# MaxMax2016/MixGAN-TTS

Hardware: AMD Instinct MI355X
Metric: denoiser steps/sec (80-mel, L=1000 frames, B=16 per GPU) (higher is better)
Workload: dtype f32

## Files before the change

include/mixgan_hip.h:

```cpp
#ifndef MIXGAN_HIP_H
#define MIXGAN_HIP_H

#include <stddef.h>
#include <stdint.h>

#ifdef __cplusplus
extern "C" {
#endif

#define MG_OK 0
#define MG_ERR_ARG (-1)
#define MG_ERR_SHAPE (-2)
#define MG_ERR_WORKSPACE (-3)

#define MG_VERSION 100

int mg_version(void);
const char *mg_error_string(int code);

#define MG_ACT_NONE 0
#define MG_ACT_RELU 1
#define MG_ACT_LRELU02 2
#define MG_ACT_TANH 3
#define MG_ACT_LRELU 4
// ... 19 lines not shown
int mg_conv1d_wgrad(const float *dy, const float *x, const float *x_vec, float *dw, float *scratch,
                    int B, int Co, int Ci, int Ldy, int Lx, int K, int stride, int pad, float alpha,
                    int accumulate, void *stream);

int mg_conv1d_wgrad_strided(const float *dy, long dy_bs, const float *x, long x_bs, const float *x_vec,
                            float *dw, float *scratch, int B, int Co, int Ci, int Ldy, int Lx, int K,
                            int stride, int pad, float alpha, int accumulate, void *stream);

size_t mg_conv1d_wgrad_grouped_scratch_floats(int Co, int Ci, int K, int G);
int mg_conv1d_wgrad_grouped(const float *dy, long dy_bs, long dy_gs, const float *x, long x_bs, long x_gs, float *dw,
                            long dw_gs, float *scratch, int G, int B, int Co, int Ci, int Ldy, int Lx, int K, int stride,
                            int pad, float alpha, int accumulate, void *stream);
int mg_conv1d_wgrad_grouped_bias(const float *dy, long dy_bs, long dy_gs, const float *x, long x_bs, long x_gs, float *dw,
                                 long dw_gs, float *db, long db_gs, float *scratch, int G, int B, int Co, int Ci, int Ldy,
                                 int Lx, int K, int stride, int pad, float alpha, int accumulate, void *stream);

int mg_rowsum(const float *in, long in_bs, int B, int R, int L, float *out_r, float *out_br,
              float alpha, int accumulate, void *stream);

int mg_conv1d_fwd_ex(const float *in, const float *in_vec, const float *packed, const float *bias,
                     const float *add, float *out, int B, int Ci, int Lin, int Co, int Lout, int K,
                     int stride, int pad, int dil, float in_slope, int act, float act_slope, float alpha,
                     int accumulate, void *stream);
int mg_conv1d_fwd_split(const float *in, const float *in_vec, const float *packed, const float *bias,
                        const float *add, float *out, int B, int Ci, int Lin, int Co, int Lout, int K, int stride,
                        int pad, int dil, float in_slope, int act, float act_slope, float alpha, int accumulate,
                        float *scratch, size_t scratch_floats, void *stream);

#define MG_CONV_EPI_PLAIN 0
#define MG_CONV_EPI_REFLECT 1
// ... 377 lines not shown
```

mixgan-tts_amd/_lib.py:

```python
import ctypes
import os
import subprocess

import torch

_HERE = os.path.dirname(os.path.abspath(__file__))
_LIB = None

class MixganHipError(RuntimeError):
    pass


MG_OK, MG_ERR_ARG, MG_ERR_SHAPE, MG_ERR_WORKSPACE = 0, -1, -2, -3
MG_ACT_NONE, MG_ACT_RELU, MG_ACT_LRELU02, MG_ACT_TANH, MG_ACT_LRELU = range(5)
MG_PACK_PLAIN, MG_PACK_GATE, MG_PACK_DGRAD, MG_PACK_TPOSE, MG_PACK_PLAIN16, MG_PACK_GATE16 = range(6)
MG_DEN_BACKWARD, MG_DEN_SPLIT, MG_DEN_P16, MG_DEN_JOBS_RESIDENT = 1, 2, 4, 8
MG_FWD_SAVE, MG_FWD_SPLIT, MG_FWD_P16 = 1, 2, 4
MG_PLAN_PER_LAYER, MG_PLAN_SINGLE = 0, 1
MG_PLAN_PERSIST, MG_PLAN_PERSIST16, MG_PLAN_TEAM16 = 0, 1, 2
MG_STATUS_TICKET, MG_STATUS_ERROR, MG_STATUS_LAUNCHES, MG_STATUS_DONE, MG_STATUS_WORDS = range(5)
MG_CONV_EPI_PLAIN, MG_CONV_EPI_REFLECT, MG_CONV_EPI_PHASES_SLICE, MG_CONV_EPI_NEEDS_WM2 = range(4)
MG_DEN_HEAD_PTRS, MG_DEN_LAYER_PTRS = 8, 9
(MG_DEN_IN_W, MG_DEN_IN_B, MG_DEN_MLP0_W, MG_DEN_MLP2_W, MG_DEN_SKIP_W, MG_DEN_SKIP_B, MG_DEN_OUT_W,
 MG_DEN_OUT_B) = range(MG_DEN_HEAD_PTRS)
# ... 18 lines not shown
                ("mel_bins", ctypes.c_int32), ("multi_speaker", ctypes.c_int32)]


class SamplingLoop(ctypes.Structure):
    _fields_ = [("cproj", ctypes.c_void_p), ("cproj_out", ctypes.c_void_p), ("step_vectors", ctypes.c_void_p),
                ("step_index", ctypes.c_int32), ("step_count", ctypes.c_int32)]


class FwdPlan(ctypes.Structure):
    _fields_ = [(n, ctypes.c_int32) for n in ("path", "family", "nt", "waves", "solo", "team", "cproj_mode", "grid",
                                              "block")]


class ConvPlan(ctypes.Structure):
    _fields_ = [(n, ctypes.c_int32) for n in ("kw", "stride", "ck", "dilmax", "mw", "wm", "nnb", "ksplit", "grid")]


def library_path():
    return os.environ.get("MG_HIP_LIB") or os.path.join(_HERE, "libmixgan_hip.so")


def build(force=False):
    if force or not os.path.exists(library_path()):
        subprocess.check_call(["make", "-C", os.path.join(_HERE, "csrc"), "-j4"] + (["-B"] if force else []))
    return library_path()


def lib():
    global _LIB
    if _LIB is None:
# ... 35 lines not shown
        "mg_conv_transpose_pack": (i, [vp, vp, i, i, i, vp]),
        "mg_conv_transpose1d_fwd": (i, [vp, vp, vp, vp, i, i, i, i, i, f, f, vp]),
        "mg_diffuse_fwd": (i, [vp] * 9 + [i, i, i, i, vp]),
        "mg_posterior_sample_fwd": (i, [vp] * 10 + [i, i, i, i, i, vp]),
        "mg_transpose_bml": (i, [vp] * 5 + [i, i, i, i, i, vp]),
        "mg_posterior_sample_bwd": (i, [vp] * 7 + [i, i, i, i, i, vp]),
        "mg_spec_affine": (i, [vp, vp, vp, vp, i, sz, i, vp]),
        "mg_conv_pack_at": (i, [vp, vp, i, i, i, i, i, i, vp]),
        "mg_conv1d_wgrad_scratch_floats": (sz, [i, i, i]),
        "mg_conv1d_wgrad": (i, [vp, vp, vp, vp, vp, i, i, i, i, i, i, i, i, f, i, vp]),
        "mg_conv1d_wgrad_strided": (i, [vp, lg, vp, lg, vp, vp, vp, i, i, i, i, i, i, i, i, f, i, vp]),
        "mg_rowsum": (i, [vp, lg, i, i, i, vp, vp, f, i, vp]),
        "mg_conv1d_wgrad_grouped_scratch_floats": (sz, [i, i, i, i]),
        "mg_conv1d_wgrad_grouped": (i, [vp, lg, lg, vp, lg, lg, vp, lg, vp, i, i, i, i, i, i, i, i, i, f, i, vp]),
        "mg_conv1d_wgrad_grouped_bias": (i, [vp, lg, lg, vp, lg, lg, vp, lg, vp, lg, vp, i, i, i, i, i, i, i, i, i, f, i, vp]),
        "mg_denoiser_packed_floats": (sz, [dp, i]),
        "mg_denoiser_pack": (i, [dp, vp, vp, vp, i, vp]),
        "mg_denoiser_bwd_workspace_floats": (sz, [dp, i, i]),
        "mg_denoiser_bwd": (i, [dp, vp, vp, vp, vp, vp, vp, vp, sz, vp, vp, vp, vp, i, i, vp]),
        "mg_denoiser_bwd_staged": (i, [dp, vp, vp, vp, vp, vp, vp, vp, sz, vp, vp, vp, vp, i, i, vp, vp]),
        "mg_denoiser_workspace_floats": (sz, [dp, i, i, i]),
        "mg_denoiser_fwd": (i, [dp, vp, vp, vp, vp, vp, vp, vp, sz, i, i, i, vp]),
        "mg_denoiser_fwd_pair": (i, [dp, vp, vp, vp, vp, vp, vp, vp, vp, vp, vp, vp, vp, sz, vp, sz, i, i, vp]),
        "mg_denoiser_fwd_plan": (i, [dp, i, i, i, i, i, ctypes.POINTER(FwdPlan)]),
        "mg_transpose_bml_strided": (i, [vp] * 5 + [i, i, i, i, i, lg, vp]),
        "mg_act_bwd": (i, [vp, vp, vp, i, sz, vp]),
        "mg_upsample_zero": (i, [vp, vp, i, i, i, i, vp]),
        "mg_step_mlp_fwd": (i, [vp] * 8 + [i, i, i, i, vp]),
        "mg_step_mlp_bwd": (i, [vp] * 8 + [i, i, i, i, vp]),
        "mg_linear_small_fwd": (i, [vp, vp, vp, i, i, i, vp]),
# ... 125 lines not shown
```

mixgan-tts_amd/autograd.py:

```python
import torch

from . import ops, _lib


def _require_cuda(*ts):
    for t in ts:
        if t is not None and not t.is_cuda:
            raise _lib.MixganHipError("tensor on %s: the HIP path has no CPU fallback" % t.device)


class _TransposeFn(torch.autograd.Function):

    @staticmethod
    def forward(ctx, x, to_blm):
        ctx.to_blm = to_blm
        return ops.transpose_bml(x.contiguous(), to_blm)

    @staticmethod
    def backward(ctx, g):
        return ops.transpose_bml(g.contiguous(), not ctx.to_blm), None


def transpose_to_bml(x):
    _require_cuda(x)
# ... 75 lines not shown
        ctx.through = through_posterior
        ctx.mark_non_differentiable(xpp) if not through_posterior else None
        return x0c, xpp

    @staticmethod
    def backward(ctx, g_x0c, g_xpp):
        x0, t, keep, c1 = ctx.saved_tensors
        g = ops.posterior_sample_bwd(x0, t, keep, c1, g_x0c.contiguous(),
                                     g_xpp.contiguous() if ctx.through else None, ctx.clip)
        return (g,) + (None,) * 9


class _Conv1dFn(torch.autograd.Function):

    @staticmethod
    def forward(ctx, x, weight, bias, in_vec, stride, padding, act):
        _require_cuda(x)
        x = x.contiguous()
        Co, Ci, K = weight.shape
        y = ops.conv1d_packed(x, ops.pack_cached(weight), None if bias is None else bias.detach(), Co, K, stride,
                              padding, act, in_vec=None if in_vec is None else in_vec.detach().contiguous(), split=True)
        ctx.save_for_backward(x, weight, y if act else None, in_vec)
        ctx.cfg = (stride, padding, act, bias is not None)
        return y

    @staticmethod
    def backward(ctx, gy):
        x, weight, y, in_vec = ctx.saved_tensors
        stride, padding, act, has_bias = ctx.cfg
        Co, Ci, K = weight.shape
        gy = gy.contiguous()
        dpre = ops.act_bwd(gy, y, act) if act else gy
        need = ctx.needs_input_grad
        vec = None if in_vec is None else in_vec.detach().contiguous()
        dw = ops.conv1d_wgrad(dpre, x, K, stride, padding, x_vec=vec) if need[1] else None
        db = ops.rowsum(dpre) if (has_bias and need[2]) else None
        dx = dvec = None
        if need[0] or (in_vec is not None and need[3]):
            Lin = x.shape[2]
            src = dpre
            if stride > 1:
                src = ops.upsample_zero(dpre, stride, (dpre.shape[2] - 1) * stride + 1)
            dx = ops.conv1d_packed(src, ops.pack_cached(weight, ops.PACK_DGRAD), None, Ci, K, 1, K - 1 - padding,
                                   Lout=Lin, split=True)
            if in_vec is not None and need[3]:
                dvec = ops.rowsum(dx, per_batch=True)
        return dx if need[0] else None, dw, db, dvec, None, None, None


def conv1d(x, weight, bias=None, stride=1, padding=0, act=None, in_vec=None):
    return _Conv1dFn.apply(x, weight, bias, in_vec, stride, padding, act)


class _StepMlpFn(torch.autograd.Function):
    @staticmethod
    def forward(ctx, t, freq, W0, W2):
        out, emb, pre, h = ops.step_mlp_fwd(t.contiguous(), freq, W0.detach().contiguous(), W2.detach().contiguous())
        ctx.save_for_backward(emb, pre, h, W2)
        return out

    @staticmethod
    def backward(ctx, g):
        emb, pre, h, W2 = ctx.saved_tensors
        dW0, dW2 = ops.step_mlp_bwd(g.contiguous(), emb, pre, h, W2.detach().contiguous())
        return None, None, dW0, dW2

# ... 189 lines not shown
```

mixgan-tts_amd/csrc/conv_api.hip:

```cpp
#include "conv_mfma.h"
#include "wgrad_mfma.h"

__global__ void pack_conv_kernel(const float *__restrict__ w, float *__restrict__ wp, PackDesc d)
{
    const size_t total = (size_t)d.MB * (d.CiP * d.K / 8) * 256;
    for (size_t idx = (size_t)blockIdx.x * blockDim.x + threadIdx.x; idx < total; idx += (size_t)gridDim.x * blockDim.x) {
        size_t dst;
        const float v = mg_pack_element(w, d, idx, &dst);
        wp[dst] = v;
    }
}

extern "C" size_t mg_conv_packed_floats(int Co, int Ci, int K, int mode)
{
    int Mrows, Kin, MB;
    if (pack_dims(Co, Ci, K, mode, &Mrows, &Kin, &MB) != MG_OK) return 0;
    const int CiP = mg_round_up(Kin, mg_conv_ck(K));
    return (size_t)MB * (CiP * K / 8) * 256;
}

extern "C" int mg_conv_pack_at(const float *w, float *packed, int Co, int Ci, int K, int mode, int q0, int Qtot,
                               void *stream)
{
    if (!w || !packed) return MG_ERR_ARG;
// ... 167 lines not shown
                               int Co, int Ci, int Ldy, int Lx, int K, int stride, int pad, float alpha,
                               int accumulate, void *stream)
{
    return mg_conv1d_wgrad_strided(dy, 0, x, 0, x_vec, dw, scratch, B, Co, Ci, Ldy, Lx, K, stride, pad, alpha, accumulate,
                                   stream);
}

__global__ __launch_bounds__(256) void rowsum_kernel(const float *__restrict__ in, long in_bs, int B, int R, int L,
                                                     float *__restrict__ out_r, float *__restrict__ out_br,
                                                     float alpha, int accumulate, int vec4)
{
    __shared__ float red[4];
    const int r = blockIdx.x;
    const int lane = threadIdx.x & 63, wave = threadIdx.x >> 6;
    if (!out_br) {
        float v = 0.f;
        if (vec4) {
            const int L4 = L >> 2;
            for (int b = 0; b < B; ++b) {
                const f32x4 *p = reinterpret_cast<const f32x4 *>(in + (size_t)b * in_bs + (size_t)r * L);
                for (int l = threadIdx.x; l < L4; l += 256) {
                    const f32x4 q = p[l];
                    v += (q[0] + q[1]) + (q[2] + q[3]);
                }
            }
        } else {
            for (int b = 0; b < B; ++b) {
                const float *p = in + (size_t)b * in_bs + (size_t)r * L;
                for (int l = threadIdx.x; l < L; l += 256) v += p[l];
            }
        }
#pragma unroll
        for (int o = 32; o > 0; o >>= 1) v += __shfl_xor(v, o, 64);
        if (lane == 0) red[wave] = v;
        __syncthreads();
        if (threadIdx.x == 0) {
            const float tot = alpha * (red[0] + red[1] + red[2] + red[3]);
            out_r[r] = accumulate ? out_r[r] + tot : tot;
        }
        return;
    }
    float tot = 0.f;
    for (int b = 0; b < B; ++b) {
        const float *p = in + (size_t)b * in_bs + (size_t)r * L;
        float v = 0.f;
        for (int l = threadIdx.x; l < L; l += 256) v += p[l];
#pragma unroll
        for (int o = 32; o > 0; o >>= 1) v += __shfl_xor(v, o, 64);
        __syncthreads();
        if (lane == 0) red[wave] = v;
        __syncthreads();
        const float s = red[0] + red[1] + red[2] + red[3];
        if (threadIdx.x == 0) out_br[(size_t)b * R + r] = alpha * s;
        tot += s;
    }
    if (out_r && threadIdx.x == 0) out_r[r] = accumulate ? out_r[r] + alpha * tot : alpha * tot;
}

extern "C" int mg_rowsum(const float *in, long in_bs, int B, int R, int L, float *out_r, float *out_br, float alpha,
                         int accumulate, void *stream)
{
    if (!in || (!out_r && !out_br)) return MG_ERR_ARG;
    if (B <= 0 || R <= 0 || L <= 0) return MG_ERR_SHAPE;
    const long bs = in_bs ? in_bs : (long)R * L;
    const int vec4 = (L % 4 == 0) && (bs % 4 == 0) && (((uintptr_t)in & 15) == 0);
    hipLaunchKernelGGL(rowsum_kernel, dim3(R), dim3(256), 0, (hipStream_t)stream, in, bs, B, R, L, out_r, out_br, alpha,
                       accumulate, vec4);
    MG_LAUNCH_CHECK();
    return MG_OK;
}
```

mixgan-tts_amd/csrc/wgrad_mfma.h:

```cpp
#pragma once
#include "common.h"
#include "wgrad_stream.h"
#include <cstdlib>

#define WG_FT 64
#define WG_RSA 65
#define WG_RSB 73

struct WgradArgs {
    const float *dy;
    const float *x;
    const float *xvec;
    float *scratch;
    long dy_bs, x_bs;
    int B, Co, Ci, Ldy, Lx, K, stride, pad;
    int chunks_per_b, nchunks, nsplit, ci_tiles;
    int G;
    long dy_gs, x_gs;
};

template <bool VEC>
__global__ __launch_bounds__(256, 2) void wgrad_mfma_kernel(WgradArgs a)
{
    __shared__ float lds[128 * WG_RSA + 128 * WG_RSB];
    float *ldsA = lds, *ldsB = lds + 128 * WG_RSA;

    const int tid = threadIdx.x;
    const int lane = tid & 63;
    const int wave = tid >> 6;
    const int wm = wave >> 1, wn = wave & 1;
    const int hh = lane >> 5, c32 = lane & 31;
    const int split = blockIdx.x;
    const int co0 = (blockIdx.y / a.ci_tiles) * 128;
    const int ci0 = (blockIdx.y % a.ci_tiles) * 128;
    const int grp = blockIdx.z / a.K;
    const int tap = blockIdx.z - grp * a.K;

    f32x16 acc[2][2];
#pragma unroll
    for (int i = 0; i < 2; ++i)
#pragma unroll
        for (int j = 0; j < 2; ++j)
#pragma unroll
            for (int r = 0; r < 16; ++r) acc[i][j][r] = 0.f;

    f32x4 va[VEC ? 8 : 1], vb[VEC ? 9 : 1];
    float sa[VEC ? 1 : 8], sb[VEC ? 1 : 8];
    const int shift = tap - a.pad;
    const int shift4 = shift & ~3, rsh = VEC ? (shift & 3) : 0;
    const int c4A = tid & 15;
    int gA[VEC ? 8 : 1], gB[VEC ? 9 : 1], lB[VEC ? 9 : 1], c4B[VEC ? 9 : 1];
// ... 120 lines not shown
    float *dst = a.scratch + (((size_t)split * a.G + grp) * a.K + tap) * a.Co * a.Ci;
#pragma unroll
    for (int i = 0; i < 2; ++i)
#pragma unroll
        for (int r = 0; r < 16; ++r) {
            const int co = co0 + wm * 64 + i * 32 + 8 * (r >> 2) + 4 * hh + (r & 3);
            if (co >= a.Co) continue;
#pragma unroll
            for (int j = 0; j < 2; ++j) {
                const int ci = ci0 + wn * 64 + j * 32 + c32;
                if (ci < a.Ci) dst[(size_t)co * a.Ci + ci] = acc[i][j][r];
            }
        }
}

__global__ __launch_bounds__(256) void wgrad_finalize_kernel(const float *__restrict__ scratch, float *__restrict__ dw,
                                                             int Co, int Ci, int K, int G, long dw_gs, int nsplit,
                                                             float alpha, int accumulate)
{
    __shared__ float part[8][32];
    const size_t per = (size_t)Co * Ci * K, n = per * G;
    const int lane = threadIdx.x & 31, grp = threadIdx.x >> 5;
    for (size_t base = (size_t)blockIdx.x * 32; base < n; base += (size_t)gridDim.x * 32) {
        const size_t i = base + lane;
        float v0 = 0.f, v1 = 0.f;
        if (i < n) {
            int s = grp;
            for (; s + 8 < nsplit; s += 16) {
                v0 += scratch[(size_t)s * n + i];
                v1 += scratch[(size_t)(s + 8) * n + i];
            }
            if (s < nsplit) v0 += scratch[(size_t)s * n + i];
        }
        part[grp][lane] = v0 + v1;
        __syncthreads();
        if (grp == 0 && i < n) {
            float v = part[0][lane];
#pragma unroll
            for (int q = 1; q < 8; ++q) v += part[q][lane];
            v *= alpha;
            const size_t g = i / per, r = i - g * per;
            const size_t cc = r % ((size_t)Co * Ci);
            const int k = (int)(r / ((size_t)Co * Ci));
            float *o = dw + g * dw_gs + cc * K + k;
            *o = accumulate ? *o + v : v;
        }
        __syncthreads();
    }
}

static inline int wgrad_nsplit(int Co, int Ci, int K, int G = 1)
{
    const int tiles = mg_cdiv(Co, 128) * mg_cdiv(Ci, 128) * K * G;
    const int target = tiles <= 8 ? 256 : 512;
    const int n = target / tiles;
    return n < 1 ? 1 : n;
}
static inline size_t wgrad_scratch_floats(int Co, int Ci, int K, int G = 1)
{
    const size_t split = (size_t)wgrad_nsplit(Co, Ci, K, G) * G * Co * Ci * K;
    const size_t stream = wgrad_stream_scratch_floats(Co, Ci, K, G);
    return split > stream ? split : stream;
}

struct WgradShape {
    int B, Co, Ci, Ldy, Lx, K, stride, pad;
    long dy_bs, x_bs;
    int G = 1;
    long dy_gs = 0, x_gs = 0, dw_gs = 0;
    float *db = nullptr;
    long db_gs = 0;
    bool *db_done = nullptr;
};

static int wgrad_launch(const WgradShape &s, const float *dy, const float *x, const float *xvec, float *dw,
                        float *scratch, float alpha, int accumulate, hipStream_t st)
{
    if (s.B <= 0 || s.Co <= 0 || s.Ci <= 0 || s.Ldy <= 0 || s.Lx <= 0 || s.K <= 0 || s.G <= 0) return MG_ERR_SHAPE;
    WgradArgs a;
    a.G = s.G;
    a.dy_gs = s.dy_gs;
    a.x_gs = s.x_gs;
    a.dy = dy;
    a.x = x;
    a.xvec = xvec;
    a.scratch = scratch;
    a.dy_bs = s.dy_bs ? s.dy_bs : (long)s.Co * s.Ldy;
    a.x_bs = s.x_bs ? s.x_bs : (long)s.Ci * s.Lx;
    a.B = s.B;
    a.Co = s.Co;
    a.Ci = s.Ci;
    a.Ldy = s.Ldy;
    a.Lx = s.Lx;
    a.K = s.K;
    a.stride = s.stride;
    a.pad = s.pad;
    a.chunks_per_b = mg_cdiv(s.Ldy, WG_FT);
    a.nchunks = a.chunks_per_b * s.B;
    a.ci_tiles = mg_cdiv(s.Ci, 128);
    int nsplit = wgrad_nsplit(s.Co, s.Ci, s.K, s.G);
    if (nsplit > a.nchunks) nsplit = a.nchunks;
    a.nsplit = nsplit;
    const size_t n = (size_t)s.Co * s.Ci * s.K * s.G;
    dim3 grid(nsplit, mg_cdiv(s.Co, 128) * a.ci_tiles, s.K * s.G);
    {
        const char *env = std::getenv("MG_WGRAD_STREAM");
        const bool stream_on = !(env && env[0] == '0');
        const long dybs = a.dy_bs, xbs = a.x_bs;
        const WsShape w = wgrad_stream_shape(s.Co, s.Ci, s.K);
        const long long units = w.cfg ? (long long)wgrad_stream_tiles(w, s.Co, s.Ci, s.G) * s.B * mg_cdiv(s.Ldy, w.FT) : 0;
        const bool ok = stream_on && w.cfg && s.stride == 1 && !xvec && s.pad == (s.K - 1) / 2 && s.Ldy == s.Lx &&
                        s.Ldy % 4 == 0 && s.Ldy >= 4 && dybs % 4 == 0 && xbs % 4 == 0 && s.dy_gs % 4 == 0 &&
                        s.x_gs % 4 == 0 && ((((uintptr_t)dy | (uintptr_t)x) & 15) == 0) && units * 2 < (1ll << 31) &&
                        units >= 8 * WS_NW;
        if (ok) {
            if (s.db_done) *s.db_done = s.db != nullptr;
            return wgrad_stream_launch(w, dy, x, dw, scratch, s.G, s.B, s.Co, s.Ci, s.Ldy, dybs, xbs, s.dy_gs, s.x_gs,
                                       s.dw_gs ? s.dw_gs : (long)s.Co * s.Ci * s.K, alpha, accumulate, st, s.db, s.db_gs);
        }
    }
    const bool vec = s.stride == 1 && !xvec && (s.Ldy % 4 == 0) && (s.Lx % 4 == 0) && (a.dy_bs % 4 == 0) &&
                     (a.x_bs % 4 == 0) && (a.dy_gs % 4 == 0) && (a.x_gs % 4 == 0) && ((((uintptr_t)dy | (uintptr_t)x) & 15) == 0) && s.Ldy >= 4 && s.Lx >= 4;
    if (vec) hipLaunchKernelGGL(wgrad_mfma_kernel<true>, grid, dim3(256), 0, st, a);
    else hipLaunchKernelGGL(wgrad_mfma_kernel<false>, grid, dim3(256), 0, st, a);
    MG_LAUNCH_CHECK();
    const int blocks = (int)((n + 31) / 32 < 8192 ? (n + 31) / 32 : 8192);
    hipLaunchKernelGGL(wgrad_finalize_kernel, dim3(blocks), dim3(256), 0, st, scratch, dw, s.Co, s.Ci, s.K, s.G,
                       s.dw_gs ? s.dw_gs : (long)s.Co * s.Ci * s.K, nsplit, alpha, accumulate);
    MG_LAUNCH_CHECK();
    return MG_OK;
}
```

mixgan-tts_amd/discriminator.py:

```python
import os

import torch
from torch import nn

from . import autograd as A
from .blocks import ConvNorm, LinearNorm, DiffusionEmbedding, Mish


class JCUDiscriminator(nn.Module):

    def __init__(self, preprocess_config, model_config, train_config):
        super().__init__()
        n_mel_channels = preprocess_config["preprocessing"]["mel"]["n_mel_channels"]
        residual_channels = model_config["denoiser"]["residual_channels"]
        dc = model_config["discriminator"]
        n_layer, n_uncond_layer, n_cond_layer = dc["n_layer"], dc["n_uncond_layer"], dc["n_cond_layer"]
        n_channels, kernel_sizes, strides = dc["n_channels"], dc["kernel_sizes"], dc["strides"]
        self.multi_speaker = model_config["multi_speaker"]

        self.input_projection = LinearNorm(2 * n_mel_channels, 2 * n_mel_channels)
        self.diffusion_embedding = DiffusionEmbedding(residual_channels)
        self.mlp = nn.Sequential(
            LinearNorm(residual_channels, residual_channels * 4),
            Mish(),
# ... 4 lines not shown

        def conv(i):
            return ConvNorm(n_channels[i - 1] if i != 0 else 2 * n_mel_channels, n_channels[i],
                            kernel_size=kernel_sizes[i], stride=strides[i], dilation=1)

        self.conv_block = nn.ModuleList([conv(i) for i in range(n_layer)])
        self.uncond_conv_block = nn.ModuleList([conv(i) for i in range(n_layer, n_layer + n_uncond_layer)])
        self.cond_conv_block = nn.ModuleList([conv(i) for i in range(n_layer, n_layer + n_cond_layer)])
        self.apply(self.weights_init)
        self._freq = None

    def weights_init(self, m):
        if m.__class__.__name__.find("ConvNorm") != -1:
            m.conv.weight.data.normal_(0.0, 0.02)

    @staticmethod
    def _lrelu_conv(layer, x, in_vec=None):
        return A.conv1d(x, layer.conv.weight, layer.conv.bias, layer.stride, layer.padding, "lrelu", in_vec)

    def forward(self, x_ts, x_t_prevs, s, t):
        dev = x_ts.device
        if self._freq is None or self._freq.device != dev:
            self._freq = self.diffusion_embedding.frequencies(dev).contiguous()
        x = A.cat_transpose(x_t_prevs, x_ts)
        x = A.conv1d(x, self.input_projection.linear.weight[:, :, None], None)
        step = A.step_mlp(t, self._freq, self.mlp[0].linear.weight, self.mlp[2].linear.weight)
        if self.multi_speaker:
            step = step + A.linear_small(s, self.spk_mlp[0].linear.weight)
        cond_feats, uncond_feats = [], []
        for layer in self.conv_block:
            x = self._lrelu_conv(layer, x)
            cond_feats.append(x)
            uncond_feats.append(x)
        x_cond, x_uncond = x, x
        overlap = (self.branch_overlap and os.environ.get("MG_JCU_OVERLAP", "1") != "0" and x.is_cuda
                   and not torch.cuda.is_current_stream_capturing())
        if overlap:
            main = torch.cuda.current_stream(dev)
            if self._side is None or self._side.device != dev:
                self._side = torch.cuda.Stream(device=dev)
# ... 22 lines not shown
```

mixgan-tts_amd/ops.py:

```python
import ctypes
import os

import torch

from . import _lib
from ._lib import fptr, iptr, check, stream_ptr

ACT = {None: _lib.MG_ACT_NONE, "none": _lib.MG_ACT_NONE, "relu": _lib.MG_ACT_RELU, "lrelu": _lib.MG_ACT_LRELU02,
       "tanh": _lib.MG_ACT_TANH, "lrelu_s": _lib.MG_ACT_LRELU}
PACK_PLAIN, PACK_GATE, PACK_DGRAD = _lib.MG_PACK_PLAIN, _lib.MG_PACK_GATE, _lib.MG_PACK_DGRAD


def pack_conv_weight(w, mode=PACK_PLAIN, out=None):
    L = _lib.lib()
    if w.dim() == 2:
        w = w[:, :, None]
    w = w.detach().contiguous()
    Co, Ci, K = w.shape
    n = L.mg_conv_packed_floats(Co, Ci, K, mode)
    if n == 0:
        raise _lib.MixganHipError("unsupported conv weight shape %s" % (tuple(w.shape),))
    if out is None or out.numel() != n or out.device != w.device:
        out = torch.empty(n, device=w.device, dtype=torch.float32)
    check(L.mg_conv_pack(fptr(w), fptr(out), Co, Ci, K, mode, stream_ptr()))
# ... 134 lines not shown
    out = torch.empty_like(x)
    check(L.mg_spec_affine(fptr(x), fptr(out), fptr(spec_min.reshape(-1)), fptr(spec_max.reshape(-1)), mode,
                           x.numel(), M, stream_ptr()))
    return out


def conv1d_wgrad(dy, x, K, stride=1, padding=0, x_vec=None, alpha=1.0):
    L = _lib.lib()
    B, Co, Ldy = dy.shape
    _, Ci, Lx = x.shape
    dw = torch.empty(Co, Ci, K, device=x.device, dtype=torch.float32)
    scratch = torch.empty(L.mg_conv1d_wgrad_scratch_floats(Co, Ci, K), device=x.device, dtype=torch.float32)
    check(L.mg_conv1d_wgrad(fptr(dy), fptr(x), fptr(x_vec, True), fptr(dw), fptr(scratch), B, Co, Ci, Ldy, Lx, K,
                            stride, padding, float(alpha), 0, stream_ptr()))
    return dw


def rowsum(x, per_batch=False, alpha=1.0):
    L = _lib.lib()
    B, R, Lf = x.shape
    out = torch.empty((B, R) if per_batch else (R,), device=x.device, dtype=torch.float32)
    check(L.mg_rowsum(fptr(x), 0, B, R, Lf, fptr(None if per_batch else out, True), fptr(out if per_batch else None, True),
                      float(alpha), 0, stream_ptr()))
    return out


def act_bwd(dy, y, act):
    L = _lib.lib()
    out = torch.empty_like(dy)
    check(L.mg_act_bwd(fptr(dy), fptr(y), fptr(out), ACT[act], dy.numel(), stream_ptr()))
# ... 254 lines not shown
```

mixgan-tts_amd/train_step.py:

```python
import os

import torch

from . import losses
from .distributed import GradBucket, ShardCounts, exchange_batch_shape, is_distributed
from .optimizer import FlatAdam


class HotPathTrainer:
    def __init__(self, diffusion, discriminator, train_config, model_config, extra_g_params=(), g_param_order=None,
                 resume=None, first_step=1, exact_shards=False):
        self.G, self.D = diffusion, discriminator
        self.exact_shards = bool(exact_shards)
        oc = train_config["optimizer"]
        self.grad_clip = oc["grad_clip_thresh"]
        self.lambda_fm = train_config["loss"]["lambda_fm" if diffusion.model != "shallow" else "lambda_fm_shallow"]
        self.n_layers = model_config["discriminator"]["n_layer"] + model_config["discriminator"]["n_cond_layer"]
        self.grad_acc = int(oc.get("grad_acc_step", 1))
        if self.grad_acc < 1:
            raise ValueError("grad_acc_step must be >= 1")
        self.step_no = int(first_step)
        g_params = list(diffusion.parameters()) + list(extra_g_params)
        self.bucketG = GradBucket(g_params, order=diffusion.denoise_fn.grad_order())
        self.bucketD = GradBucket(list(discriminator.parameters()))
        order_g = list(g_param_order) if g_param_order is not None else g_params
        if self.bucketG.flat.is_cuda:
            diffusion.denoise_fn.bind_grad_buffer(self.bucketG.flat, self.bucketG.offsets)
            self.optG = FlatAdam(self.bucketG, lr=oc["init_lr_G"], betas=oc["betas"], param_order=order_g)
            self.optD = FlatAdam(self.bucketD, lr=oc["init_lr_D"], betas=oc["betas"],
                                 param_order=list(discriminator.parameters()))
        else:
            self.optG = torch.optim.Adam(order_g, lr=oc["init_lr_G"], betas=oc["betas"])
            self.optD = torch.optim.Adam(discriminator.parameters(), lr=oc["init_lr_D"], betas=oc["betas"])
        if resume is not None:
            for mine, theirs in ((self.optG, resume[0]), (self.optD, resume[1])):
                if isinstance(mine, FlatAdam):
                    mine.adopt(theirs)
                else:
                    mine.load_state_dict(theirs.state_dict())
        self.sdlG = torch.optim.lr_scheduler.ExponentialLR(self.optG, gamma=oc["gamma"])
        self.sdlD = torch.optim.lr_scheduler.ExponentialLR(self.optD, gamma=oc["gamma"])
        if resume is not None:
            self.sdlG.load_state_dict(resume[2].state_dict())
            self.sdlD.load_state_dict(resume[3].state_dict())
        self.d_loss_fn, self.g_loss_fn = losses.get_adversarial_losses_fn(train_config["loss"]["adv_loss_mode"])
# ... 408 lines not shown
```

Before: 373.1.

## Batch discriminator conv weight-gradients into grouped multi-job MFMA kernel launches

Discriminator convolutions defer their weight and bias gradient work to a group that is flushed at the end of backward. The flush launches a single job-table MFMA wgrad kernel plus one finalize kernel that also does the bias rowsums, instead of separate wgrad and rowsum launches per layer. Gradients are written straight into the flat gradient bucket views, which saves extra allocations and copies. This removes per-layer launch overhead and raises GPU occupancy for the small wgrad problems, at the cost of extra Python bookkeeping, cross-stream waits and a deferred callback.

```diff
diff --git a/include/mixgan_hip.h b/include/mixgan_hip.h
--- a/include/mixgan_hip.h
+++ b/include/mixgan_hip.h
@@ -57,6 +57,16 @@
 int mg_conv1d_wgrad_grouped_bias(const float *dy, long dy_bs, long dy_gs, const float *x, long x_bs, long x_gs, float *dw,
                                  long dw_gs, float *db, long db_gs, float *scratch, int G, int B, int Co, int Ci, int Ldy,
                                  int Lx, int K, int stride, int pad, float alpha, int accumulate, void *stream);
+
+typedef struct mg_wgrad_job {
+    const float *dy, *x, *x_vec;
+    float *dw, *db;
+    int B, Co, Ci, Ldy, Lx, K, stride, pad;
+    float alpha;
+    int accumulate, db_accumulate;
+} mg_wgrad_job;
+size_t mg_conv1d_wgrad_jobs_scratch_floats(const mg_wgrad_job *jobs, int n);
+int mg_conv1d_wgrad_jobs(const mg_wgrad_job *jobs, int n, float *scratch, void *stream);
 
 int mg_rowsum(const float *in, long in_bs, int B, int R, int L, float *out_r, float *out_br,
               float alpha, int accumulate, void *stream);
diff --git a/mixgan-tts_amd/_lib.py b/mixgan-tts_amd/_lib.py
--- a/mixgan-tts_amd/_lib.py
+++ b/mixgan-tts_amd/_lib.py
@@ -56,6 +56,12 @@
 
 class ConvPlan(ctypes.Structure):
     _fields_ = [(n, ctypes.c_int32) for n in ("kw", "stride", "ck", "dilmax", "mw", "wm", "nnb", "ksplit", "grid")]
+
+
+class WgradJob(ctypes.Structure):
+    _fields_ = ([(n, ctypes.c_void_p) for n in ("dy", "x", "x_vec", "dw", "db")] +
+                [(n, ctypes.c_int32) for n in ("B", "Co", "Ci", "Ldy", "Lx", "K", "stride", "pad")] +
+                [("alpha", ctypes.c_float), ("accumulate", ctypes.c_int32), ("db_accumulate", ctypes.c_int32)])
 
 
 def library_path():
@@ -121,6 +127,8 @@
         "mg_conv1d_wgrad_grouped_scratch_floats": (sz, [i, i, i, i]),
         "mg_conv1d_wgrad_grouped": (i, [vp, lg, lg, vp, lg, lg, vp, lg, vp, i, i, i, i, i, i, i, i, i, f, i, vp]),
         "mg_conv1d_wgrad_grouped_bias": (i, [vp, lg, lg, vp, lg, lg, vp, lg, vp, lg, vp, i, i, i, i, i, i, i, i, i, f, i, vp]),
+        "mg_conv1d_wgrad_jobs_scratch_floats": (sz, [ctypes.POINTER(WgradJob), i]),
+        "mg_conv1d_wgrad_jobs": (i, [ctypes.POINTER(WgradJob), i, vp, vp]),
         "mg_denoiser_packed_floats": (sz, [dp, i]),
         "mg_denoiser_pack": (i, [dp, vp, vp, vp, i, vp]),
         "mg_denoiser_bwd_workspace_floats": (sz, [dp, i, i]),
diff --git a/mixgan-tts_amd/autograd.py b/mixgan-tts_amd/autograd.py
--- a/mixgan-tts_amd/autograd.py
+++ b/mixgan-tts_amd/autograd.py
@@ -113,7 +113,7 @@
 class _Conv1dFn(torch.autograd.Function):
 
     @staticmethod
-    def forward(ctx, x, weight, bias, in_vec, stride, padding, act):
+    def forward(ctx, x, weight, bias, in_vec, stride, padding, act, member=None):
         _require_cuda(x)
         x = x.contiguous()
         Co, Ci, K = weight.shape
@@ -121,6 +121,7 @@
                               padding, act, in_vec=None if in_vec is None else in_vec.detach().contiguous(), split=True)
         ctx.save_for_backward(x, weight, y if act else None, in_vec)
         ctx.cfg = (stride, padding, act, bias is not None)
+        ctx.member = member
         return y
 
     @staticmethod
@@ -132,8 +133,13 @@
         dpre = ops.act_bwd(gy, y, act) if act else gy
         need = ctx.needs_input_grad
         vec = None if in_vec is None else in_vec.detach().contiguous()
-        dw = ops.conv1d_wgrad(dpre, x, K, stride, padding, x_vec=vec) if need[1] else None
-        db = ops.rowsum(dpre) if (has_bias and need[2]) else None
+        if ctx.member is not None and need[1]:
+            group, wparam, bparam = ctx.member
+            group.add(dpre, x, vec, wparam, bparam if (has_bias and need[2]) else None, stride, padding)
+            dw = db = None
+        else:
+            dw = ops.conv1d_wgrad(dpre, x, K, stride, padding, x_vec=vec) if need[1] else None
+            db = ops.rowsum(dpre) if (has_bias and need[2]) else None
         dx = dvec = None
         if need[0] or (in_vec is not None and need[3]):
             Lin = x.shape[2]
@@ -144,11 +150,86 @@
                                    Lout=Lin, split=True)
             if in_vec is not None and need[3]:
                 dvec = ops.rowsum(dx, per_batch=True)
-        return dx if need[0] else None, dw, db, dvec, None, None, None
-
-
-def conv1d(x, weight, bias=None, stride=1, padding=0, act=None, in_vec=None):
-    return _Conv1dFn.apply(x, weight, bias, in_vec, stride, padding, act)
+        return dx if need[0] else None, dw, db, dvec, None, None, None, None
+
+
+def conv1d(x, weight, bias=None, stride=1, padding=0, act=None, in_vec=None, member=None):
+    return _Conv1dFn.apply(x, weight, bias, in_vec, stride, padding, act, member)
+
+
+class WgradGroup:
+
+    def __init__(self):
+        self.jobs = []
+
+    @staticmethod
+    def set_home(param, view):
+        param.__dict__["_mg_grad_home"] = view
+
+    def reset(self):
+        self.jobs = []
+
+    def add(self, dy, x, x_vec, wparam, bparam, stride, padding):
+        if not self.jobs:
+            torch.autograd.Variable._execution_engine.queue_callback(self.flush)
+        self.jobs.append((dy, x, x_vec, wparam, bparam, stride, padding, torch.cuda.current_stream(dy.device)))
+
+    @staticmethod
+    def _target(p):
+        g = p.grad
+        if g is None:
+            home = p.__dict__.get("_mg_grad_home")
+            if home is None or home.shape != p.shape or home.device != p.device:
+                home = torch.empty(p.shape, device=p.device, dtype=torch.float32)
+            p.grad = home
+            return home, False, None
+        if g.dtype == torch.float32 and g.is_contiguous() and g.device == p.device:
+            return g, True, None
+        tmp = torch.empty(p.shape, device=p.device, dtype=torch.float32)
+        return tmp, False, tmp
+
+    def flush(self):
+        jobs, self.jobs = self.jobs, []
+        if not jobs:
+            return
+        dev = jobs[0][0].device
+        with torch.no_grad(), torch.cuda.device(dev):
+            cur = torch.cuda.current_stream(dev)
+            waited = set()
+            for (dy, x, x_vec, _, _, _, _, stream) in jobs:
+                if stream != cur:
+                    if stream.cuda_stream not in waited and not torch.cuda.is_current_stream_capturing():
+                        cur.wait_stream(stream)
+                    waited.add(stream.cuda_stream)
+                    for t in (dy, x, x_vec):
+                        if t is not None:
+                            t.record_stream(cur)
+            waves, last = [], {}
+            for job in jobs:
+                w = 1 + max([last.get(id(p), -1) for p in job[3:5] if p is not None])
+                for p in job[3:5]:
+                    if p is not None:
+                        last[id(p)] = w
+                if w == len(waves):
+                    waves.append([])
+                waves[w].append(job)
+            for wave in waves:
+                table, later = [], []
+                for (dy, x, x_vec, wp, bp, stride, padding, _) in wave:
+                    dw, acc, add_w = self._target(wp)
+                    job = {"dy": dy, "x": x, "x_vec": x_vec, "dw": dw, "accumulate": acc, "stride": stride,
+                           "padding": padding}
+                    if add_w is not None:
+                        later.append((wp, add_w))
+                    if bp is not None:
+                        db, dacc, add_b = self._target(bp)
+                        job["db"], job["db_accumulate"] = db, dacc
+                        if add_b is not None:
+                            later.append((bp, add_b))
+                    table.append(job)
+                ops.conv1d_wgrad_jobs(table)
+                for p, t in later:
+                    p.grad = p.grad + t.to(p.grad.dtype).view_as(p.grad)
 
 
 class _StepMlpFn(torch.autograd.Function):
diff --git a/mixgan-tts_amd/csrc/conv_api.hip b/mixgan-tts_amd/csrc/conv_api.hip
--- a/mixgan-tts_amd/csrc/conv_api.hip
+++ b/mixgan-tts_amd/csrc/conv_api.hip
@@ -205,30 +205,8 @@
     const int r = blockIdx.x;
     const int lane = threadIdx.x & 63, wave = threadIdx.x >> 6;
     if (!out_br) {
-        float v = 0.f;
-        if (vec4) {
-            const int L4 = L >> 2;
-            for (int b = 0; b < B; ++b) {
-                const f32x4 *p = reinterpret_cast<const f32x4 *>(in + (size_t)b * in_bs + (size_t)r * L);
-                for (int l = threadIdx.x; l < L4; l += 256) {
-                    const f32x4 q = p[l];
-                    v += (q[0] + q[1]) + (q[2] + q[3]);
-                }
-            }
-        } else {
-            for (int b = 0; b < B; ++b) {
-                const float *p = in + (size_t)b * in_bs + (size_t)r * L;
-                for (int l = threadIdx.x; l < L; l += 256) v += p[l];
-            }
-        }
-#pragma unroll
-        for (int o = 32; o > 0; o >>= 1) v += __shfl_xor(v, o, 64);
-        if (lane == 0) red[wave] = v;
-        __syncthreads();
-        if (threadIdx.x == 0) {
-            const float tot = alpha * (red[0] + red[1] + red[2] + red[3]);
-            out_r[r] = accumulate ? out_r[r] + tot : tot;
-        }
+        const float tot = alpha * rowsum_row_total(in, in_bs, B, L, r, vec4, red);
+        if (threadIdx.x == 0) out_r[r] = accumulate ? out_r[r] + tot : tot;
         return;
     }
     float tot = 0.f;
@@ -254,9 +232,50 @@
     if (!in || (!out_r && !out_br)) return MG_ERR_ARG;
     if (B <= 0 || R <= 0 || L <= 0) return MG_ERR_SHAPE;
     const long bs = in_bs ? in_bs : (long)R * L;
-    const int vec4 = (L % 4 == 0) && (bs % 4 == 0) && (((uintptr_t)in & 15) == 0);
+    const int vec4 = rowsum_vec4(in, bs, L);
     hipLaunchKernelGGL(rowsum_kernel, dim3(R), dim3(256), 0, (hipStream_t)stream, in, bs, B, R, L, out_r, out_br, alpha,
                        accumulate, vec4);
     MG_LAUNCH_CHECK();
     return MG_OK;
 }
+
+static WgradJob wgrad_job_of(const mg_wgrad_job &j)
+{
+    return WgradJob{j.dy, j.x, j.x_vec, j.dw, j.db, j.B, j.Co, j.Ci, j.Ldy, j.Lx, j.K, j.stride, j.pad, j.alpha,
+                    j.accumulate, j.db_accumulate};
+}
+
+extern "C" size_t mg_conv1d_wgrad_jobs_scratch_floats(const mg_wgrad_job *jobs, int n)
+{
+    if (!jobs || n <= 0) return 0;
+    size_t tot = WG_TABLE_FLOATS;
+    for (int i = 0; i < n; ++i) {
+        if (jobs[i].Co <= 0 || jobs[i].Ci <= 0 || jobs[i].K <= 0) return 0;
+        tot += wgrad_job_scratch_floats(wgrad_job_of(jobs[i]));
+    }
+    return tot;
+}
+
+extern "C" int mg_conv1d_wgrad_jobs(const mg_wgrad_job *jobs, int n, float *scratch, void *stream)
+{
+    if (!jobs || !scratch) return MG_ERR_ARG;
+    if (n <= 0) return MG_ERR_SHAPE;
+    float *sc = scratch + WG_TABLE_FLOATS;
+    for (int at = 0; at < n; at += WG_MAX_JOBS) {
+        const int m = n - at < WG_MAX_JOBS ? n - at : WG_MAX_JOBS;
+        WgradJob batch[WG_MAX_JOBS];
+        float *alone[WG_MAX_JOBS];
+        for (int i = 0; i < m; ++i) batch[i] = wgrad_job_of(jobs[at + i]);
+        MG_TRY(wgrad_jobs_batch(batch, m, scratch, sc, alone, (hipStream_t)stream));
+        for (int i = 0; i < m; ++i) {
+            const WgradJob &j = batch[i];
+            if (alone[i]) {
+                MG_TRY(mg_conv1d_wgrad(j.dy, j.x, j.xvec, j.dw, alone[i], j.B, j.Co, j.Ci, j.Ldy, j.Lx, j.K, j.stride, j.pad,
+                                       j.alpha, j.accumulate, stream));
+                if (j.db) MG_TRY(mg_rowsum(j.dy, 0, j.B, j.Co, j.Ldy, j.db, nullptr, j.alpha, j.db_accumulate, stream));
+            }
+            sc += wgrad_job_scratch_floats(j);
+        }
+    }
+    return MG_OK;
+}
diff --git a/mixgan-tts_amd/csrc/wgrad_mfma.h b/mixgan-tts_amd/csrc/wgrad_mfma.h
--- a/mixgan-tts_amd/csrc/wgrad_mfma.h
+++ b/mixgan-tts_amd/csrc/wgrad_mfma.h
@@ -19,10 +19,10 @@
     long dy_gs, x_gs;
 };
 
+#define WG_LDS_FLOATS (128 * WG_RSA + 128 * WG_RSB)
 template <bool VEC>
-__global__ __launch_bounds__(256, 2) void wgrad_mfma_kernel(WgradArgs a)
-{
-    __shared__ float lds[128 * WG_RSA + 128 * WG_RSB];
+__device__ __forceinline__ void wgrad_mfma_unit(const WgradArgs &a, float *lds, const int split, const int tile, const int z)
+{
     float *ldsA = lds, *ldsB = lds + 128 * WG_RSA;
 
     const int tid = threadIdx.x;
@@ -30,11 +30,10 @@
     const int wave = tid >> 6;
     const int wm = wave >> 1, wn = wave & 1;
     const int hh = lane >> 5, c32 = lane & 31;
-    const int split = blockIdx.x;
-    const int co0 = (blockIdx.y / a.ci_tiles) * 128;
-    const int ci0 = (blockIdx.y % a.ci_tiles) * 128;
-    const int grp = blockIdx.z / a.K;
-    const int tap = blockIdx.z - grp * a.K;
+    const int co0 = (tile / a.ci_tiles) * 128;
+    const int ci0 = (tile % a.ci_tiles) * 128;
+    const int grp = z / a.K;
+    const int tap = z - grp * a.K;
 
     f32x16 acc[2][2];
 #pragma unroll
@@ -185,14 +184,21 @@
         }
 }
 
-__global__ __launch_bounds__(256) void wgrad_finalize_kernel(const float *__restrict__ scratch, float *__restrict__ dw,
-                                                             int Co, int Ci, int K, int G, long dw_gs, int nsplit,
-                                                             float alpha, int accumulate)
-{
-    __shared__ float part[8][32];
+template <bool VEC>
+__global__ __launch_bounds__(256, 2) void wgrad_mfma_kernel(WgradArgs a)
+{
+    __shared__ float lds[WG_LDS_FLOATS];
+    wgrad_mfma_unit<VEC>(a, lds, blockIdx.x, blockIdx.y, blockIdx.z);
+}
+
+__device__ __forceinline__ void wgrad_finalize_blocks(const float *__restrict__ scratch, float *__restrict__ dw, int Co,
+                                                      int Ci, int K, int G, long dw_gs, int nsplit, float alpha,
+                                                      int accumulate, float (*part)[32], const unsigned blk,
+                                                      const unsigned nblk)
+{
     const size_t per = (size_t)Co * Ci * K, n = per * G;
     const int lane = threadIdx.x & 31, grp = threadIdx.x >> 5;
-    for (size_t base = (size_t)blockIdx.x * 32; base < n; base += (size_t)gridDim.x * 32) {
+    for (size_t base = (size_t)blk * 32; base < n; base += (size_t)nblk * 32) {
         const size_t i = base + lane;
         float v0 = 0.f, v1 = 0.f;
         if (i < n) {
@@ -217,6 +223,112 @@
             *o = accumulate ? *o + v : v;
         }
         __syncthreads();
+    }
+}
+
+__global__ __launch_bounds__(256) void wgrad_finalize_kernel(const float *__restrict__ scratch, float *__restrict__ dw,
+                                                             int Co, int Ci, int K, int G, long dw_gs, int nsplit,
+                                                             float alpha, int accumulate)
+{
+    __shared__ float part[8][32];
+    wgrad_finalize_blocks(scratch, dw, Co, Ci, K, G, dw_gs, nsplit, alpha, accumulate, part, blockIdx.x, gridDim.x);
+}
+
+__device__ __forceinline__ float rowsum_row_total(const float *__restrict__ in, long in_bs, int B, int L, int r, int vec4,
+                                                  float *red)
+{
+    const int lane = threadIdx.x & 63, wave = threadIdx.x >> 6;
+    float v = 0.f;
+    if (vec4) {
+        const int L4 = L >> 2;
+        for (int b = 0; b < B; ++b) {
+            const f32x4 *p = reinterpret_cast<const f32x4 *>(in + (size_t)b * in_bs + (size_t)r * L);
+            for (int l = threadIdx.x; l < L4; l += 256) {
+                const f32x4 q = p[l];
+                v += (q[0] + q[1]) + (q[2] + q[3]);
+            }
+        }
+    } else {
+        for (int b = 0; b < B; ++b) {
+            const float *p = in + (size_t)b * in_bs + (size_t)r * L;
+            for (int l = threadIdx.x; l < L; l += 256) v += p[l];
+        }
+    }
+#pragma unroll
+    for (int o = 32; o > 0; o >>= 1) v += __shfl_xor(v, o, 64);
+    if (lane == 0) red[wave] = v;
+    __syncthreads();
+    return red[0] + red[1] + red[2] + red[3];
+}
+static inline int rowsum_vec4(const float *in, long bs, int L) { return (L % 4 == 0) && (bs % 4 == 0) && (((uintptr_t)in & 15) == 0); }
+
+#define WG_MAX_JOBS 16
+struct WgradJobDev {
+    WgradArgs a;
+    float *dw, *db;
+    float alpha;
+    int accumulate, db_accumulate, db_vec4;
+    int ytiles;
+    int fin_blocks;
+    int vec;
+};
+struct WgradJobTable {
+    int nform[3];
+    int form_job[3][WG_MAX_JOBS];
+    int form_start[3][WG_MAX_JOBS + 1];
+    int nfin;
+    int fin_start[2 * WG_MAX_JOBS + 1];
+    WgradJobDev job[WG_MAX_JOBS];
+};
+static_assert(sizeof(WgradJobTable) <= 4000, "the table travels as a kernel argument");
+#define WG_TABLE_FLOATS ((sizeof(WgradJobTable) + 255) / 256 * 64)
+
+__device__ __forceinline__ int wgrad_job_search(const int *__restrict__ start, int n, int u)
+{
+    int lo = 0, hi = n;
+    while (hi - lo > 1) {
+        const int mid = (lo + hi) >> 1;
+        if (start[mid] <= u) lo = mid;
+        else hi = mid;
+    }
+    return lo;
+}
+
+__global__ __launch_bounds__(256) void wgrad_jobs_upload_kernel(WgradJobTable t, WgradJobTable *dst)
+{
+    const int *src = reinterpret_cast<const int *>(&t);
+    int *d = reinterpret_cast<int *>(dst);
+    for (unsigned i = threadIdx.x; i < sizeof(WgradJobTable) / 4; i += 256) d[i] = src[i];
+}
+
+template <int FORM>
+__global__ __launch_bounds__(256, 2) void wgrad_mfma_jobs_kernel(const WgradJobTable *__restrict__ t)
+{
+    __shared__ float lds[WG_LDS_FLOATS];
+    const int e = wgrad_job_search(t->form_start[FORM], t->nform[FORM], (int)blockIdx.x);
+    const WgradJobDev &j = t->job[t->form_job[FORM][e]];
+    const WgradArgs a = j.a;
+    int r = (int)blockIdx.x - t->form_start[FORM][e];
+    const int split = r % a.nsplit;
+    r /= a.nsplit;
+    const int tile = r % j.ytiles;
+    if (FORM == 1 || (FORM == 2 && j.vec)) wgrad_mfma_unit<true>(a, lds, split, tile, r / j.ytiles);
+    else wgrad_mfma_unit<false>(a, lds, split, tile, r / j.ytiles);
+}
+
+__global__ __launch_bounds__(256) void wgrad_finalize_jobs_kernel(const WgradJobTable *__restrict__ t)
+{
+    __shared__ float part[8][32];
+    __shared__ float red[4];
+    const int e = wgrad_job_search(t->fin_start, t->nfin, (int)blockIdx.x);
+    const WgradJobDev &j = t->job[e >> 1];
+    const unsigned local = blockIdx.x - t->fin_start[e];
+    if (!(e & 1)) {
+        wgrad_finalize_blocks(j.a.scratch, j.dw, j.a.Co, j.a.Ci, j.a.K, 1, (long)j.a.Co * j.a.Ci * j.a.K, j.a.nsplit, j.alpha,
+                              j.accumulate, part, local, (unsigned)j.fin_blocks);
+    } else {
+        const float tot = j.alpha * rowsum_row_total(j.a.dy, j.a.dy_bs, j.a.B, j.a.Ldy, (int)local, j.db_vec4, red);
+        if (threadIdx.x == 0) j.db[local] = j.db_accumulate ? j.db[local] + tot : tot;
     }
 }
 
@@ -244,11 +356,17 @@
     bool *db_done = nullptr;
 };
 
-static int wgrad_launch(const WgradShape &s, const float *dy, const float *x, const float *xvec, float *dw,
-                        float *scratch, float alpha, int accumulate, hipStream_t st)
+enum { WG_KIND_SCALAR = 0, WG_KIND_VEC = 1, WG_KIND_STREAM = 2 };
+struct WgradPlan {
+    WgradArgs a;
+    int kind;
+    WsShape w;
+    int ytiles, z;
+};
+static int wgrad_plan(const WgradShape &s, const float *dy, const float *x, const float *xvec, float *scratch, WgradPlan *p)
 {
     if (s.B <= 0 || s.Co <= 0 || s.Ci <= 0 || s.Ldy <= 0 || s.Lx <= 0 || s.K <= 0 || s.G <= 0) return MG_ERR_SHAPE;
-    WgradArgs a;
+    WgradArgs &a = p->a;
     a.G = s.G;
     a.dy_gs = s.dy_gs;
     a.x_gs = s.x_gs;
@@ -272,8 +390,8 @@
     int nsplit = wgrad_nsplit(s.Co, s.Ci, s.K, s.G);
     if (nsplit > a.nchunks) nsplit = a.nchunks;
     a.nsplit = nsplit;
-    const size_t n = (size_t)s.Co * s.Ci * s.K * s.G;
-    dim3 grid(nsplit, mg_cdiv(s.Co, 128) * a.ci_tiles, s.K * s.G);
+    p->ytiles = mg_cdiv(s.Co, 128) * a.ci_tiles;
+    p->z = s.K * s.G;
     {
         const char *env = std::getenv("MG_WGRAD_STREAM");
         const bool stream_on = !(env && env[0] == '0');
@@ -285,19 +403,130 @@
                         s.x_gs % 4 == 0 && ((((uintptr_t)dy | (uintptr_t)x) & 15) == 0) && units * 2 < (1ll << 31) &&
                         units >= 8 * WS_NW;
         if (ok) {
-            if (s.db_done) *s.db_done = s.db != nullptr;
-            return wgrad_stream_launch(w, dy, x, dw, scratch, s.G, s.B, s.Co, s.Ci, s.Ldy, dybs, xbs, s.dy_gs, s.x_gs,
-                                       s.dw_gs ? s.dw_gs : (long)s.Co * s.Ci * s.K, alpha, accumulate, st, s.db, s.db_gs);
+            p->kind = WG_KIND_STREAM;
+            p->w = w;
+            return MG_OK;
         }
     }
     const bool vec = s.stride == 1 && !xvec && (s.Ldy % 4 == 0) && (s.Lx % 4 == 0) && (a.dy_bs % 4 == 0) &&
                      (a.x_bs % 4 == 0) && (a.dy_gs % 4 == 0) && (a.x_gs % 4 == 0) && ((((uintptr_t)dy | (uintptr_t)x) & 15) == 0) && s.Ldy >= 4 && s.Lx >= 4;
-    if (vec) hipLaunchKernelGGL(wgrad_mfma_kernel<true>, grid, dim3(256), 0, st, a);
+    p->kind = vec ? WG_KIND_VEC : WG_KIND_SCALAR;
+    return MG_OK;
+}
+static inline int wgrad_finalize_grid(size_t n) { return (int)((n + 31) / 32 < 8192 ? (n + 31) / 32 : 8192); }
+
+static int wgrad_launch(const WgradShape &s, const float *dy, const float *x, const float *xvec, float *dw,
+                        float *scratch, float alpha, int accumulate, hipStream_t st)
+{
+    WgradPlan p;
+    MG_TRY(wgrad_plan(s, dy, x, xvec, scratch, &p));
+    const WgradArgs &a = p.a;
+    if (p.kind == WG_KIND_STREAM) {
+        if (s.db_done) *s.db_done = s.db != nullptr;
+        return wgrad_stream_launch(p.w, dy, x, dw, scratch, s.G, s.B, s.Co, s.Ci, s.Ldy, a.dy_bs, a.x_bs, s.dy_gs, s.x_gs,
+                                   s.dw_gs ? s.dw_gs : (long)s.Co * s.Ci * s.K, alpha, accumulate, st, s.db, s.db_gs);
+    }
+    const size_t n = (size_t)s.Co * s.Ci * s.K * s.G;
+    dim3 grid(a.nsplit, p.ytiles, p.z);
+    if (p.kind == WG_KIND_VEC) hipLaunchKernelGGL(wgrad_mfma_kernel<true>, grid, dim3(256), 0, st, a);
     else hipLaunchKernelGGL(wgrad_mfma_kernel<false>, grid, dim3(256), 0, st, a);
     MG_LAUNCH_CHECK();
-    const int blocks = (int)((n + 31) / 32 < 8192 ? (n + 31) / 32 : 8192);
-    hipLaunchKernelGGL(wgrad_finalize_kernel, dim3(blocks), dim3(256), 0, st, scratch, dw, s.Co, s.Ci, s.K, s.G,
-                       s.dw_gs ? s.dw_gs : (long)s.Co * s.Ci * s.K, nsplit, alpha, accumulate);
+    hipLaunchKernelGGL(wgrad_finalize_kernel, dim3(wgrad_finalize_grid(n)), dim3(256), 0, st, scratch, dw, s.Co, s.Ci, s.K,
+                       s.G, s.dw_gs ? s.dw_gs : (long)s.Co * s.Ci * s.K, a.nsplit, alpha, accumulate);
     MG_LAUNCH_CHECK();
     return MG_OK;
 }
+
+struct WgradJob {
+    const float *dy, *x, *xvec;
+    float *dw, *db;
+    int B, Co, Ci, Ldy, Lx, K, stride, pad;
+    float alpha;
+    int accumulate, db_accumulate;
+};
+static inline size_t wgrad_job_scratch_floats(const WgradJob &j)
+{
+    return (wgrad_scratch_floats(j.Co, j.Ci, j.K) + 63) / 64 * 64;
+}
+static int wgrad_jobs_batch(const WgradJob *jobs, int n, float *table, float *sc, float **alone, hipStream_t st)
+{
+    WgradJobTable t{};
+    WgradJobTable *dev = reinterpret_cast<WgradJobTable *>(table);
+    int work[WG_MAX_JOBS];
+    int nj = 0;
+    for (int i = 0; i < n; ++i) {
+        const WgradJob &j = jobs[i];
+        alone[i] = nullptr;
+        if (!j.dy || !j.x || !j.dw) return MG_ERR_ARG;
+        if (j.stride < 1 || j.pad < 0) return MG_ERR_SHAPE;
+        WgradShape s{j.B, j.Co, j.Ci, j.Ldy, j.Lx, j.K, j.stride, j.pad, 0, 0};
+        WgradPlan p;
+        MG_TRY(wgrad_plan(s, j.dy, j.x, j.xvec, sc, &p));
+        if (p.kind == WG_KIND_STREAM) {
+            alone[i] = sc;
+        } else {
+            WgradJobDev &d = t.job[nj];
+            d.a = p.a;
+            d.dw = j.dw;
+            d.db = j.db;
+            d.alpha = j.alpha;
+            d.accumulate = j.accumulate;
+            d.db_accumulate = j.db_accumulate;
+            d.db_vec4 = rowsum_vec4(j.dy, p.a.dy_bs, j.Ldy);
+            d.ytiles = p.ytiles;
+            d.fin_blocks = wgrad_finalize_grid((size_t)j.Co * j.Ci * j.K);
+            d.vec = p.kind == WG_KIND_VEC;
+            work[nj] = mg_cdiv(p.a.nchunks, p.a.nsplit);
+            for (int f = d.vec; f <= 2; f += 2 - d.vec) {
+                int at = t.nform[f]++;
+                while (at > 0 && work[t.form_job[f][at - 1]] < work[nj]) {
+                    t.form_job[f][at] = t.form_job[f][at - 1];
+                    --at;
+                }
+                t.form_job[f][at] = nj;
+            }
+            ++nj;
+        }
+        sc += wgrad_job_scratch_floats(j);
+    }
+    if (nj == 0) return MG_OK;
+    long long tot = 0;
+    for (int f = 0; f < 3; ++f) {
+        long long u = 0;
+        for (int e = 0; e < t.nform[f]; ++e) {
+            const WgradJobDev &d = t.job[t.form_job[f][e]];
+            t.form_start[f][e] = (int)u;
+            u += (long long)d.a.nsplit * d.ytiles * d.a.K;
+        }
+        if (u >= (1ll << 31)) return MG_ERR_SHAPE;
+        t.form_start[f][t.nform[f]] = (int)u;
+    }
+    t.nfin = 2 * nj;
+    for (int e = 0; e < nj; ++e) {
+        t.fin_start[2 * e] = (int)tot;
+        tot += t.job[e].fin_blocks;
+        t.fin_start[2 * e + 1] = (int)tot;
+        tot += t.job[e].db ? t.job[e].a.Co : 0;
+    }
+    if (tot >= (1ll << 31)) return MG_ERR_SHAPE;
+    t.fin_start[2 * nj] = (int)tot;
+    hipLaunchKernelGGL(wgrad_jobs_upload_kernel, dim3(1), dim3(256), 0, st, t, dev);
+    MG_LAUNCH_CHECK();
+    const char *env = std::getenv("MG_WGRAD_JOBS_GRIDS");
+    if (!(env && env[0] == '2') && t.nform[0] && t.nform[1]) {
+        hipLaunchKernelGGL(wgrad_mfma_jobs_kernel<2>, dim3(t.form_start[2][nj]), dim3(256), 0, st, dev);
+        MG_LAUNCH_CHECK();
+    } else {
+        if (t.nform[0]) {
+            hipLaunchKernelGGL(wgrad_mfma_jobs_kernel<0>, dim3(t.form_start[0][t.nform[0]]), dim3(256), 0, st, dev);
+            MG_LAUNCH_CHECK();
+        }
+        if (t.nform[1]) {
+            hipLaunchKernelGGL(wgrad_mfma_jobs_kernel<1>, dim3(t.form_start[1][t.nform[1]]), dim3(256), 0, st, dev);
+            MG_LAUNCH_CHECK();
+        }
+    }
+    hipLaunchKernelGGL(wgrad_finalize_jobs_kernel, dim3((unsigned)tot), dim3(256), 0, st, dev);
+    MG_LAUNCH_CHECK();
+    return MG_OK;
+}
diff --git a/mixgan-tts_amd/discriminator.py b/mixgan-tts_amd/discriminator.py
--- a/mixgan-tts_amd/discriminator.py
+++ b/mixgan-tts_amd/discriminator.py
@@ -42,16 +42,31 @@
         if m.__class__.__name__.find("ConvNorm") != -1:
             m.conv.weight.data.normal_(0.0, 0.02)
 
-    @staticmethod
-    def _lrelu_conv(layer, x, in_vec=None):
-        return A.conv1d(x, layer.conv.weight, layer.conv.bias, layer.stride, layer.padding, "lrelu", in_vec)
+    def _lrelu_conv(self, layer, x, in_vec=None):
+        conv = layer.conv
+        return A.conv1d(x, conv.weight, conv.bias, layer.stride, layer.padding, "lrelu", in_vec,
+                        self._member(conv.weight, conv.bias))
+
+    wgrad_group = True
+    _group = None
+    _grouping = False
+
+    def _member(self, weight, bias):
+        return (self._group, weight, bias) if self._grouping else None
 
     def forward(self, x_ts, x_t_prevs, s, t):
         dev = x_ts.device
         if self._freq is None or self._freq.device != dev:
             self._freq = self.diffusion_embedding.frequencies(dev).contiguous()
+        self._grouping = (self.wgrad_group and os.environ.get("MG_WGRAD_GROUP", "1") != "0" and x_ts.is_cuda
+                          and torch.is_grad_enabled())
+        if self._grouping:
+            if self._group is None:
+                self._group = A.WgradGroup()
+            self._group.reset()
         x = A.cat_transpose(x_t_prevs, x_ts)
-        x = A.conv1d(x, self.input_projection.linear.weight[:, :, None], None)
+        w_in = self.input_projection.linear.weight
+        x = A.conv1d(x, w_in[:, :, None], None, member=self._member(w_in, None))
         step = A.step_mlp(t, self._freq, self.mlp[0].linear.weight, self.mlp[2].linear.weight)
         if self.multi_speaker:
             step = step + A.linear_small(s, self.spk_mlp[0].linear.weight)
diff --git a/mixgan-tts_amd/ops.py b/mixgan-tts_amd/ops.py
--- a/mixgan-tts_amd/ops.py
+++ b/mixgan-tts_amd/ops.py
@@ -172,6 +172,39 @@
     check(L.mg_conv1d_wgrad(fptr(dy), fptr(x), fptr(x_vec, True), fptr(dw), fptr(scratch), B, Co, Ci, Ldy, Lx, K,
                             stride, padding, float(alpha), 0, stream_ptr()))
     return dw
+
+
+_JOBS_SCRATCH = {}
+
+
+def conv1d_wgrad_jobs(jobs):
+    L = _lib.lib()
+    n = len(jobs)
+    if n == 0:
+        return
+    arr = (_lib.WgradJob * n)()
+    for a, j in zip(arr, jobs):
+        dy, x, dw = j["dy"], j["x"], j["dw"]
+        B, Co, Ldy = dy.shape
+        _, Ci, Lx = x.shape
+        if dw.numel() % (Co * Ci) or x.shape[0] != B:
+            raise _lib.MixganHipError("conv1d_wgrad_jobs: dw %s does not belong to dy %s, x %s" %
+                                      (tuple(dw.shape), tuple(dy.shape), tuple(x.shape)))
+        db = j.get("db")
+        if db is not None and db.numel() != Co:
+            raise _lib.MixganHipError("conv1d_wgrad_jobs: db has %d elements for %d channels" % (db.numel(), Co))
+        a.dy, a.x, a.x_vec = fptr(dy).value, fptr(x).value, fptr(j.get("x_vec"), True).value
+        a.dw, a.db = fptr(dw).value, fptr(db, True).value
+        a.B, a.Co, a.Ci, a.Ldy, a.Lx, a.K = B, Co, Ci, Ldy, Lx, dw.numel() // (Co * Ci)
+        a.stride, a.pad, a.alpha = j.get("stride", 1), j.get("padding", 0), float(j.get("alpha", 1.0))
+        a.accumulate, a.db_accumulate = int(bool(j.get("accumulate"))), int(bool(j.get("db_accumulate")))
+    dev = jobs[0]["dy"].device
+    need = L.mg_conv1d_wgrad_jobs_scratch_floats(arr, n)
+    key = (dev, torch.cuda.current_stream(dev).cuda_stream)
+    scratch = _JOBS_SCRATCH.get(key)
+    if scratch is None or scratch.numel() < need:
+        scratch = _JOBS_SCRATCH[key] = torch.empty(need, device=dev, dtype=torch.float32)
+    check(L.mg_conv1d_wgrad_jobs(arr, n, fptr(scratch), stream_ptr()))
 
 
 def rowsum(x, per_batch=False, alpha=1.0):
diff --git a/mixgan-tts_amd/train_step.py b/mixgan-tts_amd/train_step.py
--- a/mixgan-tts_amd/train_step.py
+++ b/mixgan-tts_amd/train_step.py
@@ -3,6 +3,7 @@
 import torch
 
 from . import losses
+from .autograd import WgradGroup
 from .distributed import GradBucket, ShardCounts, exchange_batch_shape, is_distributed
 from .optimizer import FlatAdam
 
@@ -29,6 +30,8 @@
             self.optG = FlatAdam(self.bucketG, lr=oc["init_lr_G"], betas=oc["betas"], param_order=order_g)
             self.optD = FlatAdam(self.bucketD, lr=oc["init_lr_D"], betas=oc["betas"],
                                  param_order=list(discriminator.parameters()))
+            for p, v in zip(self.bucketD.params, self.bucketD.views):
+                WgradGroup.set_home(p, v)
         else:
             self.optG = torch.optim.Adam(order_g, lr=oc["init_lr_G"], betas=oc["betas"])
             self.optD = torch.optim.Adam(discriminator.parameters(), lr=oc["init_lr_D"], betas=oc["betas"])
```

Result: no change. 372.8 (-0.1%).
